# jiaw-z/DKT-Stereo

Hardware: AMD Instinct MI355X
Metric: stereo pairs/sec at 736x1248 D=192, 32 iters (RAFT-Stereo test_mode forward) (higher is better)
Workload: dtype f32 io/accumulate; convolution products = 3x fp16-split MFMA (22-bit operands); lookup / correlation exact fp32

## Files before the change

### dkt_stereo_amd/csrc/corr_feat.hip

```cpp
#include "dkt_common.h"
#include <cstdlib>
#include <type_traits>

typedef float cf_f32x16 __attribute__((ext_vector_type(16)));

struct CorrFeatArgs {
    DktPtrs skew;
    const float *coords_x;
    long coords_bstride;
    const float *w;
    const float *bias;
    float *out;
    long out_bstride;
    float *tap;
    long tap_bstride;
    long HW;
    int H, W1, W2, pitch, nseg, Cout, relu;
    float inv_wm1[DKT_MAX_LEVELS];
    char *out_c8;
    long out_c8_bs, out_c8_plane;
    int out_c8_Wp, out_c8_ch0;
    float act_scale;
};

// ... 178 lines not shown
    const long waves = (long)a.H * a.nseg;
    dim3 grid((unsigned)((waves + 3) / 4), (unsigned)B);
    if (a.Cout <= 32) hipLaunchKernelGGL((corr_feat_kernel<L, R, 1>), grid, dim3(256), 0, st, a);
    else hipLaunchKernelGGL((corr_feat_kernel<L, R, 2>), grid, dim3(256), 0, st, a);
    return dkt_launch_status();
}

typedef float cf_f32x4 __attribute__((ext_vector_type(4)));

template <int R, int MT>
__global__ __launch_bounds__(256) void corr_feat16_kernel(CorrFeatArgs a) {
    constexpr int K = 2 * R + 1;
    const int lane = threadIdx.x & 63;
    const int li = lane & 15, g = lane >> 4;
    const long gw = blockIdx.x * 4L + (threadIdx.x >> 6);
    const long hrow = gw / a.nseg;
    if (hrow >= a.H) return;
    const int seg0 = (int)(gw - hrow * a.nseg) * 16;
    const int w1 = seg0 + li;
    const bool live = w1 < a.W1;
    const int w1c = live ? w1 : a.W1 - 1;
    const int b = blockIdx.y;
    const long p = hrow * a.W1 + w1c;
    const float cx = a.coords_x[(size_t)b * a.coords_bstride + p];

    float A[MT][K];
#pragma unroll
    for (int s = 0; s < K; ++s)
#pragma unroll
        for (int m = 0; m < MT; ++m) {
            const int co = 16 * m + li;
            const bool ok = co < a.Cout;
            const float wv = a.w[(long)(g * K + s) * a.Cout + (ok ? co : 0)];
            A[m][s] = ok ? wv : 0.0f;
        }
    float bv[MT][4];
#pragma unroll
    for (int m = 0; m < MT; ++m)
#pragma unroll
        for (int r = 0; r < 4; ++r) bv[m][r] = 0.0f;
    if (a.bias) {
#pragma unroll
        for (int m = 0; m < MT; ++m)
#pragma unroll
            for (int r = 0; r < 4; ++r) {
                const int co = 16 * m + 4 * g + r;
                bv[m][r] = a.bias[co < a.Cout ? co : a.Cout - 1];
            }
    }

    const int lv = g;
    const int wi = a.W2 >> lv;
    const int qm = (w1c >> lv) % wi;
    const float *lvl = g == 0 ? a.skew.p[0] : g == 1 ? a.skew.p[1] : g == 2 ? a.skew.p[2] : a.skew.p[3];
    const float inv = g == 0 ? a.inv_wm1[0] : g == 1 ? a.inv_wm1[1] : g == 2 ? a.inv_wm1[2] : a.inv_wm1[3];
    const float *base = lvl + (((long)b * a.H + hrow) * wi) * (long)a.pitch + w1c;
    const float xc = __fdiv_rn(cx, (float)(1 << lv));
    const float wm1 = (float)(wi - 1);
    const float hwm1 = __fdiv_rn(wm1, 2.0f);
    DktTap taps[K];
#pragma unroll
    for (int k = 0; k < K; ++k) taps[k] = cf_tap(__fadd_rn((float)(k - R), xc), wm1, inv, hwm1);
    const int i0 = cf_clamp_idx(taps[0].fl, wi);
    float win[K + 1];
#pragma unroll
    for (int t = 0; t <= K; ++t) {
        const int c = i0 + t;
        const bool in = c >= 0 && c < wi;
        int sidx = (in ? c : 0) - qm;
        if (sidx < 0) sidx += wi;
        const float x = base[(long)sidx * a.pitch];
        win[t] = in ? x : 0.0f;
    }
    bool odd = false;
#pragma unroll
    for (int k = 0; k < K; ++k) odd |= cf_clamp_idx(taps[k].fl, wi) != i0 + k;
    float v[K];
#pragma unroll
    for (int k = 0; k < K; ++k) v[k] = dkt_blend(win[k], win[k + 1], taps[k]);
    if (__any(odd)) {
        auto at = [&](int c) -> float {
            if (c < 0 || c >= wi) return 0.0f;
            int sidx = c - qm;
            if (sidx < 0) sidx += wi;
            return base[(long)sidx * a.pitch];
        };
#pragma unroll
        for (int k = 0; k < K; ++k) {
            const int ik = cf_clamp_idx(taps[k].fl, wi);
            if (ik != i0 + k) v[k] = dkt_blend(at(ik), at(ik + 1), taps[k]);
        }
    }
    if (a.tap && live) {
        float *t = a.tap + (size_t)b * a.tap_bstride + p;
#pragma unroll
        for (int k = 0; k < K; ++k) t[(size_t)(g * K + k) * a.HW] = v[k];
    }

    cf_f32x4 acc[MT];
#pragma unroll
    for (int m = 0; m < MT; ++m)
#pragma unroll
        for (int r = 0; r < 4; ++r) {
            acc[m][r] = 0.0f;
            asm volatile("" ::"v"(bv[m][r]));
        }
#pragma unroll
    for (int s = 0; s < K; ++s)
#pragma unroll
        for (int m = 0; m < MT; ++m)
            acc[m] = __builtin_amdgcn_mfma_f32_16x16x4f32(A[m][s], v[s], acc[m], 0, 0, 0);

    const bool full = 16 * MT <= a.Cout && seg0 + 16 <= a.W1;
    if (a.out_c8) {
        char *pb = a.out_c8 + (size_t)b * a.out_c8_bs + ((size_t)(hrow + 1) * a.out_c8_Wp + (w1c + 1)) * 16;
#pragma unroll
        for (int m = 0; m < MT; ++m) {
            unsigned hw[2], lw[2];
#pragma unroll
            for (int d = 0; d < 2; ++d) {
                float y0 = __fadd_rn(acc[m][2 * d], bv[m][2 * d]), y1 = __fadd_rn(acc[m][2 * d + 1], bv[m][2 * d + 1]);
                if (a.relu) { y0 = dkt_relu(y0); y1 = dkt_relu(y1); }
                if (16 * m + 4 * g + 2 * d >= a.Cout) y0 = 0.0f;
                if (16 * m + 4 * g + 2 * d + 1 >= a.Cout) y1 = 0.0f;
                y0 *= a.act_scale; y1 *= a.act_scale;
                const _Float16 h0 = (_Float16)y0, h1 = (_Float16)y1;
                union { _Float16 h[2]; unsigned u; } t0, t1;
                t0.h[0] = h0; t0.h[1] = h1;
                t1.h[0] = (_Float16)(y0 - (float)h0); t1.h[1] = (_Float16)(y1 - (float)h1);
                hw[d] = t0.u; lw[d] = t1.u;
            }
            const bool even = (g & 1) == 0;
            const unsigned s0 = __shfl_xor(even ? lw[0] : hw[0], 16), s1 = __shfl_xor(even ? lw[1] : hw[1], 16);
            const uint4 v = even ? make_uint4(hw[0], hw[1], s0, s1) : make_uint4(s0, s1, lw[0], lw[1]);
            if (live) {
                const int grp = ((a.out_c8_ch0 + 16 * m) >> 3) + (g >> 1);
                *(uint4 *)(pb + (size_t)grp * 2 * a.out_c8_plane + (even ? 0 : a.out_c8_plane)) = v;
            }
        }
        return;
    }
    float *ob = a.out + (size_t)b * a.out_bstride + hrow * a.W1 + w1c;
#pragma unroll
    for (int m = 0; m < MT; ++m)
#pragma unroll
        for (int r = 0; r < 4; ++r) {
            const int co = 16 * m + 4 * g + r;
            float y = __fadd_rn(acc[m][r], bv[m][r]);
            if (a.relu) y = dkt_relu(y);
            if (full || (co < a.Cout && live)) ob[(size_t)co * a.HW] = y;
        }
}

template <int R, class CX>
__device__ __forceinline__ void corr_feat64_body(const CorrFeatArgs &a, long bx, int b, CX coord) {
    constexpr int K = 2 * R + 1;
    constexpr int VP = 12;
    static_assert((4 * K + 3) / 4 <= VP, "row pitch holds the k steps");
    __shared__ __attribute__((aligned(16))) float vs[4 * 64 * VP];
    const int lane = threadIdx.x & 63;
    const int g = __builtin_amdgcn_readfirstlane(threadIdx.x >> 6);
    const int nseg = (a.W1 + 63) / 64;
    const long hrow = bx / nseg;
    const int seg0 = (int)(bx - hrow * nseg) * 64;
    constexpr int NS = (4 * K) / 4;
    float Aw[NS];
    {
        const int j = lane & 15, q = lane >> 4;
        const int co = 16 * g + j;
#pragma unroll
        for (int sidx = 0; sidx < NS; ++sidx) {
            const int kk = 4 * sidx + q;
            const float wv = a.w[(long)kk * a.Cout + (co < a.Cout ? co : 0)];
            Aw[sidx] = co < a.Cout ? wv : 0.0f;
        }
    }
    {
        const int w1 = seg0 + lane;
        const bool live = w1 < a.W1;
        const int w1c = live ? w1 : a.W1 - 1;
        const long p = hrow * a.W1 + w1c;
        const float cx = coord(b, p, live, g);
        const int lv = g;
        const int wi = a.W2 >> lv;
        const int qm = (w1c >> lv) % wi;
        const float *lvl = a.skew.p[lv];
        const float inv = a.inv_wm1[lv];
        const float *base = lvl + (((long)b * a.H + hrow) * wi) * (long)a.pitch + w1c;
        const float xc = __fdiv_rn(cx, (float)(1 << lv));
        const float wm1 = (float)(wi - 1);
        const float hwm1 = __fdiv_rn(wm1, 2.0f);
        DktTap taps[K];
#pragma unroll
        for (int k = 0; k < K; ++k) taps[k] = cf_tap(__fadd_rn((float)(k - R), xc), wm1, inv, hwm1);
        const int i0 = cf_clamp_idx(taps[0].fl, wi);
        float win[K + 1];
#pragma unroll
        for (int t = 0; t <= K; ++t) {
            const int c = i0 + t;
            const bool in = c >= 0 && c < wi;
            int sidx = (in ? c : 0) - qm;
            if (sidx < 0) sidx += wi;
            const float x = base[(long)sidx * a.pitch];
            win[t] = in ? x : 0.0f;
        }
        bool odd = false;
#pragma unroll
        for (int k = 0; k < K; ++k) odd |= cf_clamp_idx(taps[k].fl, wi) != i0 + k;
        float v[K];
#pragma unroll
        for (int k = 0; k < K; ++k) v[k] = dkt_blend(win[k], win[k + 1], taps[k]);
        if (__any(odd)) {
            auto at = [&](int c) -> float {
                if (c < 0 || c >= wi) return 0.0f;
                int sidx = c - qm;
                if (sidx < 0) sidx += wi;
                return base[(long)sidx * a.pitch];
            };
#pragma unroll
            for (int k = 0; k < K; ++k) {
                const int ik = cf_clamp_idx(taps[k].fl, wi);
                if (ik != i0 + k) v[k] = dkt_blend(at(ik), at(ik + 1), taps[k]);
            }
        }
#pragma unroll
        for (int k = 0; k < K; ++k) vs[(((g * K + k) & 3) * 64 + lane) * VP + ((g * K + k) >> 2)] = v[k];
        if (a.tap && live) {
            float *t = a.tap + (size_t)b * a.tap_bstride + p;
#pragma unroll
            for (int k = 0; k < K; ++k) t[(size_t)(g * K + k) * a.HW] = v[k];
        }
    }
    __syncthreads();
    const int m = g;
    if (16 * m >= a.Cout) return;
    const int j = lane & 15, q = lane >> 4;
    typedef float f32x4_ __attribute__((ext_vector_type(4)));
    f32x4_ acc[4];
#pragma unroll
    for (int t = 0; t < 4; ++t) acc[t] = f32x4_{0.f, 0.f, 0.f, 0.f};
#pragma unroll
    for (int t0 = 0; t0 < 4; t0 += 2) {
        float bs[2][VP];
#pragma unroll
        for (int t = 0; t < 2; ++t) {
            const float4 *row = (const float4 *)(vs + (q * 64 + 16 * (t0 + t) + j) * VP);
#pragma unroll
            for (int i = 0; i < VP / 4; ++i) {
                const float4 f = row[i];
                bs[t][4 * i] = f.x; bs[t][4 * i + 1] = f.y; bs[t][4 * i + 2] = f.z; bs[t][4 * i + 3] = f.w;
            }
        }
#pragma unroll
        for (int sidx = 0; sidx < NS; ++sidx) {
#pragma unroll
            for (int t = 0; t < 2; ++t) acc[t0 + t] = __builtin_amdgcn_mfma_f32_16x16x4f32(Aw[sidx], bs[t][sidx], acc[t0 + t], 0, 0, 0);
        }
    }
    float bv[4];
#pragma unroll
    for (int r = 0; r < 4; ++r) {
        const int co = 16 * m + 4 * q + r;
        bv[r] = a.bias ? a.bias[co < a.Cout ? co : a.Cout - 1] : 0.0f;
    }
#pragma unroll
    for (int t = 0; t < 4; ++t) {
        const int w1 = seg0 + 16 * t + j;
        const bool live = w1 < a.W1;
        float y[4];
#pragma unroll
        for (int r = 0; r < 4; ++r) {
            y[r] = __fadd_rn(acc[t][r], bv[r]);
            if (a.relu) y[r] = dkt_relu(y[r]);
            if (16 * m + 4 * q + r >= a.Cout) y[r] = 0.0f;
        }
        if (a.out_c8) {
            unsigned hw[2], lw[2];
#pragma unroll
            for (int d = 0; d < 2; ++d) {
                const float y0 = y[2 * d] * a.act_scale, y1 = y[2 * d + 1] * a.act_scale;
                const _Float16 h0 = (_Float16)y0, h1 = (_Float16)y1;
                union { _Float16 h[2]; unsigned u; } t0, t1;
                t0.h[0] = h0; t0.h[1] = h1;
                t1.h[0] = (_Float16)(y0 - (float)h0); t1.h[1] = (_Float16)(y1 - (float)h1);
                hw[d] = t0.u; lw[d] = t1.u;
            }
            const bool even = (q & 1) == 0;
            const unsigned s0 = __shfl_xor(even ? lw[0] : hw[0], 16), s1 = __shfl_xor(even ? lw[1] : hw[1], 16);
            const uint4 v = even ? make_uint4(hw[0], hw[1], s0, s1) : make_uint4(s0, s1, lw[0], lw[1]);
            if (live) {
                const int grp = ((a.out_c8_ch0 + 16 * m) >> 3) + (q >> 1);
                char *pb = a.out_c8 + (size_t)b * a.out_c8_bs + ((size_t)(hrow + 1) * a.out_c8_Wp + (w1 + 1)) * 16;
                *(uint4 *)(pb + (size_t)grp * 2 * a.out_c8_plane + (even ? 0 : a.out_c8_plane)) = v;
            }
        } else if (live) {
            float *ob = a.out + (size_t)b * a.out_bstride + hrow * a.W1 + w1;
#pragma unroll
            for (int r = 0; r < 4; ++r) {
                const int co = 16 * m + 4 * q + r;
                if (co < a.Cout) ob[(size_t)co * a.HW] = y[r];
            }
        }
    }
}

template <int R>
__global__ __launch_bounds__(256, 8) void corr_feat64_kernel(CorrFeatArgs a) {
    corr_feat64_body<R>(a, (long)blockIdx.x, (int)blockIdx.y,
                        [&](int b, long p, bool, int) -> float { return a.coords_x[(size_t)b * a.coords_bstride + p]; });
}

#include "stem7_body.h"

struct FrontArgs {
    CorrFeatArgs cf;
    Stem7Args s7;
    const float *planes; long planes_bs; int n_co;
    const float *head_bias;
    const float *x_old; long x_old_bs;
    float *x_new; long x_new_bs;
    const float *x0; long x0_bs;
    float *flow; long flow_bs;
    int nb_stem;
};

__device__ __forceinline__ float front_coord(const FrontArgs &f, int b, int oh, int ow, long p) {
    const int H = f.cf.H, W = f.cf.W1;
    const long HW = f.cf.HW;
    float s = 0.0f;
    for (int cb = 0; cb < f.n_co; ++cb) {
        const float *pl = f.planes + (long)b * f.planes_bs + (long)cb * 9 * HW;
#pragma unroll
        for (int t = 0; t < 9; ++t) {
            const int ih = oh + t / 3 - 1, iw = ow + t % 3 - 1;
            const bool in = ih >= 0 && ih < H && iw >= 0 && iw < W;
            const float v = pl[(long)t * HW + (in ? (long)ih * W + iw : 0)];
            s = __fadd_rn(s, in ? v : 0.0f);
        }
    }
    s = __fadd_rn(s, f.head_bias ? f.head_bias[0] : 0.0f);
    return __fadd_rn(f.x_old[(long)b * f.x_old_bs + p], s);
}

template <int R>
__global__ __launch_bounds__(256) void motion_front_kernel(FrontArgs f) {
    const int b = blockIdx.y;
    if ((int)blockIdx.x < f.nb_stem) {
        const long HW = f.cf.HW;
        const float *fl = f.flow + (long)b * f.flow_bs;
        const float *x0 = f.x0 + (long)b * f.x0_bs;
        stem7_tile(f.s7, (int)(blockIdx.x / f.s7.n_co), (int)(blockIdx.x % f.s7.n_co), b, [&](int ih, int iw, long off, float (&v)[4]) {
            v[0] = __fsub_rn(front_coord(f, b, ih, iw, off), x0[off]);
#pragma unroll
            for (int c = 1; c < 4; ++c) v[c] = fl[(long)(c < f.s7.Cin ? c : 0) * HW + off];
        });
        return;
    }
    corr_feat64_body<R>(f.cf, (long)blockIdx.x - f.nb_stem, b, [&](int bb, long p, bool live, int g) -> float {
        const int oh = (int)(p / f.cf.W1), ow = (int)(p - (long)oh * f.cf.W1);
        const float nx = front_coord(f, bb, oh, ow, p);
        if (g == 0 && live) {
            f.x_new[(long)bb * f.x_new_bs + p] = nx;
            f.flow[(long)bb * f.flow_bs + p] = __fsub_rn(nx, f.x0[(long)bb * f.x0_bs + p]);
        }
        return nx;
    });
}

template <int R>
static int cf16_launch(CorrFeatArgs a, int B, hipStream_t st) {
    a.nseg = (a.W1 + 15) / 16;
    const long waves = (long)a.H * a.nseg;
    dim3 grid((unsigned)((waves + 3) / 4), (unsigned)B);
    switch ((a.Cout + 15) / 16) {
        case 1: hipLaunchKernelGGL((corr_feat16_kernel<R, 1>), grid, dim3(256), 0, st, a); break;
        case 2: hipLaunchKernelGGL((corr_feat16_kernel<R, 2>), grid, dim3(256), 0, st, a); break;
        case 3: hipLaunchKernelGGL((corr_feat16_kernel<R, 3>), grid, dim3(256), 0, st, a); break;
        default: hipLaunchKernelGGL((corr_feat16_kernel<R, 4>), grid, dim3(256), 0, st, a); break;
    }
    return dkt_launch_status();
}

static int corr_feat_impl(const float *const *skew, const float *coords_x, long coords_bstride,
                          const float *weight, const float *bias, float *out, long out_bstride,
                          float *tap, long tap_bstride, void *out_c8, long out_c8_bstride_bytes, int out_c8_ch0, float act_scale,
                          int B, int H, int W1, int W2, int L, int r, int Cout, int relu,
                          int device, void *stream) {
    if (!skew || !coords_x || !weight || (!out && !out_c8)) return DKT_E_NULL;
    if (out_c8 && (L != 4 || (out_c8_ch0 & 7) || !(act_scale > 0.0f))) return DKT_E_UNSUPPORTED;
    if (B <= 0 || H <= 0 || W1 <= 0 || W2 <= 0 || B > 65535 || Cout <= 0) return DKT_E_SHAPE;
    if (L < 1 || L > DKT_MAX_LEVELS || (W2 >> (L - 1)) == 0) return DKT_E_LEVELS;
    if (r < 0 || r > DKT_MAX_RADIUS) return DKT_E_RADIUS;
    if (Cout > 64 || !((L == 4 || L == 2 || L == 3) && (r == 4 || r == 3))) return DKT_E_UNSUPPORTED;
    if ((W2 >> (L - 1)) < 2) return DKT_E_UNSUPPORTED;
    CorrFeatArgs a;
    for (int i = 0; i < DKT_MAX_LEVELS; ++i) {
        a.skew.p[i] = i < L ? skew[i] : nullptr;
        if (i < L && !skew[i]) return DKT_E_NULL;
        const int wi = i < L ? (W2 >> i) : 0;
        a.inv_wm1[i] = wi > 1 ? (float)(1.0 / (double)(wi - 1)) : 0.0f;
    }
    a.coords_x = coords_x;
    a.coords_bstride = coords_bstride;
    a.w = weight;
    a.bias = bias;
    a.out = out;
    a.out_bstride = out_bstride;
    a.tap = tap;
    a.tap_bstride = tap_bstride;
    a.HW = (long)H * W1;
    a.H = H; a.W1 = W1; a.W2 = W2;
    a.pitch = (W1 + 31) & ~31;
    a.nseg = (W1 + 31) / 32;
    a.Cout = Cout;
    a.relu = relu ? 1 : 0;
    int Hp = 0, Wp = 0;
    dkt_act_c8_dims(H, W1, &Hp, &Wp);
    a.out_c8 = (char *)out_c8; a.out_c8_bs = out_c8_bstride_bytes; a.out_c8_plane = (long)Hp * Wp * 16;
    a.out_c8_Wp = Wp; a.out_c8_ch0 = out_c8_ch0; a.act_scale = act_scale;
    DKT_ENTER(device);
    hipStream_t st = (hipStream_t)stream;
    if (L == 4) {
        const long blocks = (long)H * ((W1 + 63) / 64);
        if (blocks > 0x7fffffffL) return DKT_E_SHAPE;
        dim3 grid((unsigned)blocks, (unsigned)B);
        if (r == 4) hipLaunchKernelGGL(corr_feat64_kernel<4>, grid, dim3(256), 0, st, a);
        else hipLaunchKernelGGL(corr_feat64_kernel<3>, grid, dim3(256), 0, st, a);
        return dkt_launch_status();
    }
    if (out_c8) return r == 4 ? cf16_launch<4>(a, B, st) : cf16_launch<3>(a, B, st);
    if (r == 4) {
        if (L == 4) return cf_launch<4, 4>(a, B, st);
        if (L == 3) return cf_launch<3, 4>(a, B, st);
        return cf_launch<2, 4>(a, B, st);
    }
    if (L == 4) return cf_launch<4, 3>(a, B, st);
    if (L == 3) return cf_launch<3, 3>(a, B, st);
    return cf_launch<2, 3>(a, B, st);
}

extern "C" int dkt_corr1d_lookup_conv1x1(const float *const *skew, const float *coords_x, long coords_bstride,
                                         const float *weight, const float *bias, float *out, long out_bstride,
                                         float *tap, long tap_bstride,
                                         int B, int H, int W1, int W2, int L, int r, int Cout, int relu,
                                         int device, void *stream) {
    if (!out) return DKT_E_NULL;
    return corr_feat_impl(skew, coords_x, coords_bstride, weight, bias, out, out_bstride, tap, tap_bstride, nullptr, 0, 0, 1.0f,
                          B, H, W1, W2, L, r, Cout, relu, device, stream);
}

extern "C" int dkt_corr1d_lookup_conv1x1_c8(const float *const *skew, const float *coords_x, long coords_bstride,
                                            const float *weight, const float *bias, void *out_c8, long out_c8_bstride_bytes,
                                            int out_c8_ch0, float act_scale, int B, int H, int W1, int W2, int L, int r, int Cout,
                                            int relu, int device, void *stream) {
    if (!out_c8) return DKT_E_NULL;
    return corr_feat_impl(skew, coords_x, coords_bstride, weight, bias, nullptr, 0, nullptr, 0, out_c8, out_c8_bstride_bytes,
                          out_c8_ch0, act_scale, B, H, W1, W2, L, r, Cout, relu, device, stream);
}

extern "C" int dkt_motion_front_c8(const dkt_motion_front_desc *d, int device, void *stream) {
    if (!d) return DKT_E_NULL;
    if (!d->skew || !d->planes || !d->x_old || !d->x_new || !d->x0 || !d->flow || !d->w_cor || !d->cor_c8 || !d->stem_w_hi ||
        !d->stem_w_lo || !d->flo_c8)
        return DKT_E_NULL;
    if (d->x_new == d->x_old) return DKT_E_SHAPE;
    const int B = d->B, H = d->H, W1 = d->W1, W2 = d->W2, L = d->L, r = d->r;
    if (B <= 0 || H <= 0 || W1 <= 0 || W2 <= 0 || B > 65535 || d->n_co < 1) return DKT_E_SHAPE;
    if (L != 4 || (r != 4 && r != 3) || d->cor_channels <= 0 || d->cor_channels > 64 || (W2 >> (L - 1)) < 2) return DKT_E_UNSUPPORTED;
    if (d->stem_cin < 1 || d->stem_cin > 4 || d->stem_cout <= 0) return DKT_E_SHAPE;
    if ((d->cor_c8_ch0 & 7) || (d->flo_c8_ch0 & 7) || !(d->cor_act_scale > 0.0f) || !(d->flo_act_scale > 0.0f) ||
        !(d->stem_in_scale > 0.0f) || !(d->stem_out_scale > 0.0f))
        return DKT_E_SHAPE;
    FrontArgs f;
    CorrFeatArgs &a = f.cf;
    for (int i = 0; i < DKT_MAX_LEVELS; ++i) {
        a.skew.p[i] = i < L ? d->skew[i] : nullptr;
        if (i < L && !d->skew[i]) return DKT_E_NULL;
        const int wi = i < L ? (W2 >> i) : 0;
        a.inv_wm1[i] = wi > 1 ? (float)(1.0 / (double)(wi - 1)) : 0.0f;
    }
    a.coords_x = nullptr; a.coords_bstride = 0;
    a.w = d->w_cor; a.bias = d->b_cor;
    a.out = nullptr; a.out_bstride = 0; a.tap = nullptr; a.tap_bstride = 0;
    a.HW = (long)H * W1;
    a.H = H; a.W1 = W1; a.W2 = W2;
    a.pitch = (W1 + 31) & ~31;
    a.nseg = (W1 + 31) / 32;
    a.Cout = d->cor_channels;
    a.relu = 1;
    int Hp = 0, Wp = 0;
    dkt_act_c8_dims(H, W1, &Hp, &Wp);
    a.out_c8 = (char *)d->cor_c8; a.out_c8_bs = d->cor_c8_bstride_bytes; a.out_c8_plane = (long)Hp * Wp * 16;
    a.out_c8_Wp = Wp; a.out_c8_ch0 = d->cor_c8_ch0; a.act_scale = d->cor_act_scale;
    Stem7Args &s = f.s7;
    s.x = nullptr; s.x_bs = 0;
    s.whi = (const _Float16 *)d->stem_w_hi; s.wlo = (const _Float16 *)d->stem_w_lo;
    s.bias = d->stem_bias; s.out_scale = d->stem_out_scale; s.in_scale = d->stem_in_scale;
    s.y = nullptr; s.y_bs = 0;
    s.Cin = d->stem_cin; s.Cout = d->stem_cout; s.CoutPad = (d->stem_cout + 63) & ~63;
    s.H = H; s.W = W1;
    s.tiles_w = (W1 + 31) / 32;
    s.tiles_xy = s.tiles_w * ((H + 3) / 4);
    s.n_co = s.CoutPad / 64;
    s.relu = 1;
    s.y_c8 = (char *)d->flo_c8; s.y_c8_bs = d->flo_c8_bstride_bytes; s.y_c8_plane = (long)Hp * Wp * 16; s.y_c8_Wp = Wp;
    s.y_c8_ch0 = d->flo_c8_ch0; s.act_scale = d->flo_act_scale;
    f.planes = d->planes; f.planes_bs = d->planes_bstride; f.n_co = d->n_co;
    f.head_bias = d->head_bias;
    f.x_old = d->x_old; f.x_old_bs = d->x_old_bstride;
    f.x_new = d->x_new; f.x_new_bs = d->x_new_bstride;
    f.x0 = d->x0; f.x0_bs = d->x0_bstride;
    f.flow = d->flow; f.flow_bs = d->flow_bstride;
    const long nb_stem = (long)s.tiles_xy * s.n_co, nb_look = (long)H * ((W1 + 63) / 64);
    if (nb_stem + nb_look > 0x7fffffffL) return DKT_E_SHAPE;
    f.nb_stem = (int)nb_stem;
    DKT_ENTER(device);
    dim3 grid((unsigned)(nb_stem + nb_look), (unsigned)B);
    if (r == 4) hipLaunchKernelGGL(motion_front_kernel<4>, grid, dim3(256), 0, (hipStream_t)stream, f);
    else hipLaunchKernelGGL(motion_front_kernel<3>, grid, dim3(256), 0, (hipStream_t)stream, f);
// ... 3 lines not shown
```

### dkt_stereo_amd/csrc/resample_c8.hip

```cpp
#include "resample.h"

__device__ __forceinline__ unsigned rs_pack_h2(_Float16 a, _Float16 b) {
    union { _Float16 h[2]; unsigned u; } v;
    v.h[0] = a;
    v.h[1] = b;
    return v.u;
}

__device__ __forceinline__ void rs_store_c8(char *p, long plane, const float (&v)[8], float scale) {
    unsigned hw[4], lw[4];
#pragma unroll
    for (int d = 0; d < 4; ++d) {
        const float x0 = v[2 * d] * scale, x1 = v[2 * d + 1] * scale;
        const _Float16 a0 = (_Float16)x0, a1 = (_Float16)x1;
        hw[d] = rs_pack_h2(a0, a1);
        lw[d] = rs_pack_h2((_Float16)(x0 - (float)a0), (_Float16)(x1 - (float)a1));
    }
    *(uint4 *)p = make_uint4(hw[0], hw[1], hw[2], hw[3]);
    *(uint4 *)(p + plane) = make_uint4(lw[0], lw[1], lw[2], lw[3]);
}

__device__ __forceinline__ void pool2x_c8_body(const float *__restrict__ x, long x_bs, char *__restrict__ dst, long dst_bs,
                                               int C, int H, int W, int Ho, int Wo, int Wp, long plane, int ch0, float scale,
                                               int bx, int oy, int bz) {
    const int ox = bx * 128 + threadIdx.x;
    const int g = bz % ((C + 7) / 8), b = bz / ((C + 7) / 8);
    if (ox >= Wo) return;
    const float *xb = x + (long)b * x_bs;
    float v[8];
#pragma unroll
    for (int k = 0; k < 8; ++k) {
        const int c = g * 8 + k;
        float t[9];
        dkt_pool9_load(xb + (long)(c < C ? c : C - 1) * H * W, H, W, oy, ox, t);
        const float avg = dkt_pool9_avg(t);
        v[k] = c < C ? avg : 0.0f;
    }
    rs_store_c8(dst + (long)b * dst_bs + (long)((ch0 >> 3) + g) * 2 * plane + ((long)(oy + 1) * Wp + (ox + 1)) * 16, plane, v, scale);
}

__device__ __forceinline__ void interp_c8_body(const float *__restrict__ x, long x_bs, char *__restrict__ dst, long dst_bs,
                                               int C, int H, int W, int Ho, int Wo, float sy, float sx, int Wp, long plane,
                                               int ch0, float scale, int bx, int oy, int bz) {
    const int ox = bx * 128 + threadIdx.x;
    const int g = bz % ((C + 7) / 8), b = bz / ((C + 7) / 8);
    if (ox >= Wo) return;
    const DktLerp ty = dkt_lerp(oy, sy, H), tx = dkt_lerp(ox, sx, W);
    const float *xb = x + (long)b * x_bs;
    float a0[8], a1[8], b0[8], b1[8];
#pragma unroll
    for (int k = 0; k < 8; ++k) {
        const int c = g * 8 + k;
        const float *p = xb + (long)(c < C ? c : C - 1) * H * W;
        a0[k] = p[(long)ty.i0 * W + tx.i0]; a1[k] = p[(long)ty.i0 * W + tx.i1];
        b0[k] = p[(long)ty.i1 * W + tx.i0]; b1[k] = p[(long)ty.i1 * W + tx.i1];
    }
    float v[8];
#pragma unroll
    for (int k = 0; k < 8; ++k) {
        const float o = dkt_lerp_blend(ty, tx, a0[k], a1[k], b0[k], b1[k]);
        v[k] = g * 8 + k < C ? o : 0.0f;
    }
    rs_store_c8(dst + (long)b * dst_bs + (long)((ch0 >> 3) + g) * 2 * plane + ((long)(oy + 1) * Wp + (ox + 1)) * 16, plane, v, scale);
}

__global__ __launch_bounds__(128) void pool2x_c8_kernel(const float *__restrict__ x, long x_bs, char *__restrict__ dst, long dst_bs,
                                                        int C, int H, int W, int Ho, int Wo, int Wp, long plane, int ch0, float scale) {
    pool2x_c8_body(x, x_bs, dst, dst_bs, C, H, W, Ho, Wo, Wp, plane, ch0, scale, blockIdx.x, blockIdx.y, blockIdx.z);
}

__global__ __launch_bounds__(128) void interp_c8_kernel(const float *__restrict__ x, long x_bs, char *__restrict__ dst, long dst_bs,
                                                        int C, int H, int W, int Ho, int Wo, float sy, float sx, int Wp, long plane,
                                                        int ch0, float scale) {
    interp_c8_body(x, x_bs, dst, dst_bs, C, H, W, Ho, Wo, sy, sx, Wp, plane, ch0, scale, blockIdx.x, blockIdx.y, blockIdx.z);
}

struct RsJob {
    const float *x; long x_bs;
    char *dst; long dst_bs;
    int C, H, W, Ho, Wo, Wp; long plane; int ch0; float scale;
    float sy, sx;
    int kind;
    int nbx, nby;
};
struct RsPair { RsJob j[2]; };

__global__ __launch_bounds__(128) void resample_pair_c8_kernel(RsPair a, int nb0) {
    const bool second = (int)blockIdx.x >= nb0;
    const RsJob &j = a.j[second ? 1 : 0];
    int id = (int)blockIdx.x - (second ? nb0 : 0);
    const int bx = id % j.nbx; id /= j.nbx;
    const int oy = id % j.nby, bz = id / j.nby;
    if (j.kind == 0) pool2x_c8_body(j.x, j.x_bs, j.dst, j.dst_bs, j.C, j.H, j.W, j.Ho, j.Wo, j.Wp, j.plane, j.ch0, j.scale, bx, oy, bz);
    else interp_c8_body(j.x, j.x_bs, j.dst, j.dst_bs, j.C, j.H, j.W, j.Ho, j.Wo, j.sy, j.sx, j.Wp, j.plane, j.ch0, j.scale, bx, oy, bz);
}

static int rs_fill(RsJob &j, const dkt_resample_c8_job *d, long &blocks) {
    if (!d || !d->x || !d->dst) return DKT_E_NULL;
    if (d->B <= 0 || d->C <= 0 || d->H <= 0 || d->W <= 0 || (d->ch0 & 7) || !(d->scale > 0.0f)) return DKT_E_SHAPE;
    if (d->kind != 0 && d->kind != 1) return DKT_E_UNSUPPORTED;
    j.x = d->x; j.x_bs = d->x_bstride; j.dst = (char *)d->dst; j.dst_bs = d->dst_bstride_bytes;
    j.C = d->C; j.H = d->H; j.W = d->W; j.ch0 = d->ch0; j.scale = d->scale; j.kind = d->kind;
    if (d->kind == 0) {
        j.Ho = (d->H - 1) / 2 + 1; j.Wo = (d->W - 1) / 2 + 1;
        j.sy = j.sx = 0.0f;
    } else {
        if (d->Ho <= 0 || d->Wo <= 0) return DKT_E_SHAPE;
        j.Ho = d->Ho; j.Wo = d->Wo;
        j.sy = j.Ho > 1 ? (float)(d->H - 1) / (float)(j.Ho - 1) : 0.0f;
        j.sx = j.Wo > 1 ? (float)(d->W - 1) / (float)(j.Wo - 1) : 0.0f;
    }
    int Hp, Wp;
    dkt_act_c8_dims(j.Ho, j.Wo, &Hp, &Wp);
    j.Wp = Wp; j.plane = (long)Hp * Wp * 16;
    j.nbx = (j.Wo + 127) / 128; j.nby = j.Ho;
    blocks = (long)j.nbx * j.nby * d->B * ((d->C + 7) / 8);
    return DKT_OK;
}

extern "C" int dkt_resample_pair_c8(const dkt_resample_c8_job *job0, const dkt_resample_c8_job *job1, int device, void *stream) {
    RsPair a;
    long n0 = 0, n1 = 0;
    int rc = rs_fill(a.j[0], job0, n0);
    if (rc != DKT_OK) return rc;
    rc = rs_fill(a.j[1], job1, n1);
    if (rc != DKT_OK) return rc;
    if (n0 + n1 > 0x7fffffffL) return DKT_E_SHAPE;
    DKT_ENTER(device);
    hipLaunchKernelGGL(resample_pair_c8_kernel, dim3((unsigned)(n0 + n1)), dim3(128), 0, (hipStream_t)stream, a, (int)n0);
    return dkt_launch_status();
}

extern "C" int dkt_pool2x_c8(const float *x, long x_bstride, void *dst, long dst_bstride_bytes, int B, int C, int H, int W,
                             int ch0, float scale, int device, void *stream) {
    if (!x || !dst) return DKT_E_NULL;
    if (B <= 0 || C <= 0 || H <= 0 || W <= 0 || (ch0 & 7) || !(scale > 0.0f)) return DKT_E_SHAPE;
    const int Ho = (H - 1) / 2 + 1, Wo = (W - 1) / 2 + 1;
    int Hp, Wp;
    dkt_act_c8_dims(Ho, Wo, &Hp, &Wp);
    const long gz = (long)B * ((C + 7) / 8);
    if (gz > 65535 || Ho > 65535) return DKT_E_SHAPE;
    DKT_ENTER(device);
    hipLaunchKernelGGL(pool2x_c8_kernel, dim3((unsigned)((Wo + 127) / 128), (unsigned)Ho, (unsigned)gz), dim3(128), 0, (hipStream_t)stream,
                       x, x_bstride, (char *)dst, dst_bstride_bytes, C, H, W, Ho, Wo, Wp, (long)Hp * Wp * 16, ch0, scale);
    return dkt_launch_status();
}

extern "C" int dkt_interp_c8(const float *x, long x_bstride, void *dst, long dst_bstride_bytes, int B, int C, int H, int W,
                             int Ho, int Wo, int ch0, float scale, int device, void *stream) {
    if (!x || !dst) return DKT_E_NULL;
    if (B <= 0 || C <= 0 || H <= 0 || W <= 0 || Ho <= 0 || Wo <= 0 || (ch0 & 7) || !(scale > 0.0f)) return DKT_E_SHAPE;
    int Hp, Wp;
    dkt_act_c8_dims(Ho, Wo, &Hp, &Wp);
    const long gz = (long)B * ((C + 7) / 8);
    if (gz > 65535 || Ho > 65535) return DKT_E_SHAPE;
    const float sy = Ho > 1 ? (float)(H - 1) / (float)(Ho - 1) : 0.0f;
    const float sx = Wo > 1 ? (float)(W - 1) / (float)(Wo - 1) : 0.0f;
    DKT_ENTER(device);
    hipLaunchKernelGGL(interp_c8_kernel, dim3((unsigned)((Wo + 127) / 128), (unsigned)Ho, (unsigned)gz), dim3(128), 0, (hipStream_t)stream,
                       x, x_bstride, (char *)dst, dst_bstride_bytes, C, H, W, Ho, Wo, sy, sx, Wp, (long)Hp * Wp * 16, ch0, scale);
    return dkt_launch_status();
}
```

### dkt_stereo_amd/csrc/stem7_body.h

```cpp
#pragma once
#include "dkt_common.h"

typedef _Float16 s7_f16x8 __attribute__((ext_vector_type(8)));
typedef _Float16 s7_f16x4 __attribute__((ext_vector_type(4)));
typedef float s7_f32x16 __attribute__((ext_vector_type(16)));

#define S7_STEPS 14

struct Stem7Args {
    const float *x;
    long x_bs;
    const _Float16 *whi, *wlo;
    const float *bias;
    float out_scale, in_scale;
    float *y;
    long y_bs;
    int Cin, Cout, CoutPad, H, W, tiles_w, tiles_xy, n_co;
    int relu;
    char *y_c8;
    long y_c8_bs, y_c8_plane;
    int y_c8_Wp, y_c8_ch0;
    float act_scale;
};

template <class LD>
__device__ __forceinline__ void stem7_tile(const Stem7Args &a, int t, int cb, int b, LD load) {
    constexpr int TR = 4, PR = TR + 6, PC = 40;
    __shared__ __attribute__((aligned(16))) _Float16 phi[PR * PC * 4], plo[PR * PC * 4];
    const int tid = threadIdx.x, lane = tid & 63, wave = tid >> 6;
    const int li = lane & 31, kg = lane >> 5;
    const int w0 = (t % a.tiles_w) * 32, h0 = (t / a.tiles_w) * TR;
    const long HW = (long)a.H * a.W;
    for (int pp = tid; pp < PR * PC; pp += 256) {
        const int pr = pp / PC, pc = pp - pr * PC;
        const int ih = h0 - 3 + pr, iw = w0 - 3 + pc;
        const bool ok = ih >= 0 && ih < a.H && iw >= 0 && iw < a.W;
        const long off = ok ? (long)ih * a.W + iw : 0;
        s7_f16x4 hv, lv;
        float in[4];
        load(ok ? ih : 0, ok ? iw : 0, off, in);
#pragma unroll
        for (int c = 0; c < 4; ++c) {
            float v = (ok && c < a.Cin) ? in[c] : 0.0f;
            v *= a.in_scale;
            const _Float16 h = (_Float16)v;
            hv[c] = h;
            lv[c] = (_Float16)(v - (float)h);
        }
        *(s7_f16x4 *)(phi + pp * 4) = hv;
        *(s7_f16x4 *)(plo + pp * 4) = lv;
    }
    __syncthreads();
    s7_f32x16 acc[2];
#pragma unroll
    for (int m = 0; m < 2; ++m)
#pragma unroll
        for (int r = 0; r < 16; ++r) acc[m][r] = 0.0f;
    const int co0 = cb * 64;
    const _Float16 *wh = a.whi + ((long)(co0 + li)) * 16 + kg * 8;
    const _Float16 *wl = a.wlo + ((long)(co0 + li)) * 16 + kg * 8;
    const long wstep = (long)a.CoutPad * 16;
#pragma unroll
    for (int s = 0; s < S7_STEPS; ++s) {
        const int dy = s >> 1, half = s & 1;
        s7_f16x8 Ah[2], Al[2];
#pragma unroll
        for (int m = 0; m < 2; ++m) {
            Ah[m] = *(const s7_f16x8 *)(wh + s * wstep + m * 32 * 16);
            Al[m] = *(const s7_f16x8 *)(wl + s * wstep + m * 32 * 16);
        }
        const int pp = (wave + dy) * PC + li + 4 * half + 2 * kg;
        union { s7_f16x8 v; s7_f16x4 h[2]; } Bh, Bl;
        Bh.h[0] = *(const s7_f16x4 *)(phi + pp * 4);
        Bh.h[1] = *(const s7_f16x4 *)(phi + pp * 4 + 4);
        Bl.h[0] = *(const s7_f16x4 *)(plo + pp * 4);
        Bl.h[1] = *(const s7_f16x4 *)(plo + pp * 4 + 4);
#pragma unroll
        for (int m = 0; m < 2; ++m) {
            acc[m] = __builtin_amdgcn_mfma_f32_32x32x16_f16(Ah[m], Bh.v, acc[m], 0, 0, 0);
            acc[m] = __builtin_amdgcn_mfma_f32_32x32x16_f16(Al[m], Bh.v, acc[m], 0, 0, 0);
            acc[m] = __builtin_amdgcn_mfma_f32_32x32x16_f16(Ah[m], Bl.v, acc[m], 0, 0, 0);
        }
    }
    const int oh = h0 + wave, ow = w0 + li;
    const bool inside = oh < a.H && ow < a.W;
    float *yo = a.y ? a.y + (long)b * a.y_bs + (long)(inside ? oh : 0) * a.W + (inside ? ow : 0) : nullptr;
#pragma unroll
    for (int m = 0; m < 2; ++m) {
        float v[16];
#pragma unroll
        for (int r = 0; r < 16; ++r) {
            const int co = co0 + m * 32 + 4 * kg + (r & 3) + 8 * (r >> 2);
            float t = acc[m][r] * a.out_scale + (a.bias ? a.bias[co < a.Cout ? co : a.Cout - 1] : 0.0f);
            if (a.relu) t = dkt_relu(t);
            v[r] = co < a.Cout ? t : 0.0f;
            if (yo && inside && co < a.Cout) yo[(long)co * HW] = v[r];
        }
        if (a.y_c8) {
#pragma unroll
            for (int jp = 0; jp < 2; ++jp) {
                unsigned ha[2], la[2], hb[2], lb[2];
#pragma unroll
                for (int d = 0; d < 2; ++d) {
                    const float x0 = v[8 * jp + 2 * d] * a.act_scale, x1 = v[8 * jp + 2 * d + 1] * a.act_scale;
                    const float y0 = v[8 * jp + 4 + 2 * d] * a.act_scale, y1 = v[8 * jp + 4 + 2 * d + 1] * a.act_scale;
                    const _Float16 a0 = (_Float16)x0, a1 = (_Float16)x1, b0 = (_Float16)y0, b1 = (_Float16)y1;
                    union { _Float16 h[2]; unsigned u; } t0, t1, t2, t3;
                    t0.h[0] = a0; t0.h[1] = a1;
                    t1.h[0] = (_Float16)(x0 - (float)a0); t1.h[1] = (_Float16)(x1 - (float)a1);
                    t2.h[0] = b0; t2.h[1] = b1;
                    t3.h[0] = (_Float16)(y0 - (float)b0); t3.h[1] = (_Float16)(y1 - (float)b1);
                    ha[d] = t0.u; la[d] = t1.u; hb[d] = t2.u; lb[d] = t3.u;
                }
#pragma unroll
                for (int d = 0; d < 2; ++d) {
                    auto r = __builtin_amdgcn_permlane32_swap(ha[d], hb[d], false, false);
                    ha[d] = r[0]; hb[d] = r[1];
                    auto q = __builtin_amdgcn_permlane32_swap(la[d], lb[d], false, false);
                    la[d] = q[0]; lb[d] = q[1];
                }
                if (inside) {
                    const int g = ((a.y_c8_ch0 + co0 + m * 32) >> 3) + 2 * jp + kg;
                    char *p = a.y_c8 + (long)b * a.y_c8_bs + (long)g * 2 * a.y_c8_plane + ((long)(oh + 1) * a.y_c8_Wp + (ow + 1)) * 16;
                    *(uint4 *)p = make_uint4(ha[0], ha[1], hb[0], hb[1]);
                    *(uint4 *)(p + a.y_c8_plane) = make_uint4(la[0], la[1], lb[0], lb[1]);
                }
            }
        }
    }
}
```

Measured before the change: 33.52.

## Share front-kernel LDS, split coord conv across waves, vectorize pool resample

In motion_front_kernel, the 3x3 plane-sum coordinate computation is now split across the four waves, with each wave loading a subset of taps into shared memory before every wave sums them. Before this, every wave recomputed all taps on its own. The stem patch and the corr sample buffer now use a single shared LDS allocation, and occupancy is hinted with launch_bounds(256,5). The resample pool kernel gains a float4-vectorized path that produces two outputs per thread, and both resample kernels now use flat 1D chunked indexing. The cost of this is added __syncthreads barriers in the corr path and extra code paths for aligned and unaligned inputs.

```diff
diff --git a/dkt_stereo_amd/csrc/corr_feat.hip b/dkt_stereo_amd/csrc/corr_feat.hip
--- a/dkt_stereo_amd/csrc/corr_feat.hip
+++ b/dkt_stereo_amd/csrc/corr_feat.hip
@@ -354,12 +354,12 @@
         }
 }
 
+#define CF64_VS_FLOATS (4 * 64 * 12)
 template <int R, class CX>
-__device__ __forceinline__ void corr_feat64_body(const CorrFeatArgs &a, long bx, int b, CX coord) {
+__device__ __forceinline__ void corr_feat64_body(const CorrFeatArgs &a, long bx, int b, CX coord, float *vs) {
     constexpr int K = 2 * R + 1;
     constexpr int VP = 12;
-    static_assert((4 * K + 3) / 4 <= VP, "row pitch holds the k steps");
-    __shared__ __attribute__((aligned(16))) float vs[4 * 64 * VP];
+    static_assert((4 * K + 3) / 4 <= VP && 4 * 64 * VP == CF64_VS_FLOATS, "row pitch holds the k steps");
     const int lane = threadIdx.x & 63;
     const int g = __builtin_amdgcn_readfirstlane(threadIdx.x >> 6);
     const int nseg = (a.W1 + 63) / 64;
@@ -382,7 +382,7 @@
         const bool live = w1 < a.W1;
         const int w1c = live ? w1 : a.W1 - 1;
         const long p = hrow * a.W1 + w1c;
-        const float cx = coord(b, p, live, g);
+        const float cx = coord(b, p, live, g, vs);
         const int lv = g;
         const int wi = a.W2 >> lv;
         const int qm = (w1c >> lv) % wi;
@@ -508,8 +508,9 @@
 
 template <int R>
 __global__ __launch_bounds__(256, 8) void corr_feat64_kernel(CorrFeatArgs a) {
+    __shared__ __attribute__((aligned(16))) float vs[CF64_VS_FLOATS];
     corr_feat64_body<R>(a, (long)blockIdx.x, (int)blockIdx.y,
-                        [&](int b, long p, bool, int) -> float { return a.coords_x[(size_t)b * a.coords_bstride + p]; });
+                        [&](int b, long p, bool, int, float *) -> float { return a.coords_x[(size_t)b * a.coords_bstride + p]; }, vs);
 }
 
 #include "stem7_body.h"
@@ -544,8 +545,49 @@
     return __fadd_rn(f.x_old[(long)b * f.x_old_bs + p], s);
 }
 
+#define FRONT_CB 4
+static_assert(FRONT_CB * 9 * 64 <= CF64_VS_FLOATS, "a pass fits the sample buffer of corr_feat64_body");
+
+__device__ __forceinline__ float front_coord_block(const FrontArgs &f, int b, long p, int g, float *vs) {
+    const int H = f.cf.H, W = f.cf.W1, lane = threadIdx.x & 63;
+    const long HW = f.cf.HW;
+    const int oh = (int)(p / W), ow = (int)(p - (long)oh * W);
+    const float xo = f.x_old[(long)b * f.x_old_bs + p];
+    const float hb = f.head_bias ? f.head_bias[0] : 0.0f;
+    float s = 0.0f;
+    for (int cb0 = 0; cb0 < f.n_co; cb0 += FRONT_CB) {
+        const int ncb = f.n_co - cb0 < FRONT_CB ? f.n_co - cb0 : FRONT_CB;
+        const float *pl = f.planes + (long)b * f.planes_bs + (long)cb0 * 9 * HW;
+        float u[FRONT_CB * 9 / 4];
+#pragma unroll
+        for (int j = 0; j < FRONT_CB * 9 / 4; ++j) {
+            const int i = g + 4 * j;
+            const int t = i % 9;
+            const int ih = oh + t / 3 - 1, iw = ow + t % 3 - 1;
+            const bool in = i < ncb * 9 && ih >= 0 && ih < H && iw >= 0 && iw < W;
+            const float v = pl[(long)(i < ncb * 9 ? i : 0) * HW + (in ? (long)ih * W + iw : 0)];
+            u[j] = in ? v : 0.0f;
+        }
+#pragma unroll
+        for (int j = 0; j < FRONT_CB * 9 / 4; ++j) vs[(g + 4 * j) * 64 + lane] = u[j];
+        __syncthreads();
+        for (int cb = 0; cb < ncb; ++cb) {
+            float t[9];
+#pragma unroll
+            for (int k = 0; k < 9; ++k) t[k] = vs[(cb * 9 + k) * 64 + lane];
+#pragma unroll
+            for (int k = 0; k < 9; ++k) s = __fadd_rn(s, t[k]);
+        }
+        __syncthreads();
+    }
+    s = __fadd_rn(s, hb);
+    return __fadd_rn(xo, s);
+}
+
 template <int R>
-__global__ __launch_bounds__(256) void motion_front_kernel(FrontArgs f) {
+__global__ __launch_bounds__(256, 5) void motion_front_kernel(FrontArgs f) {
+    static_assert(S7_PATCH_HALVES * 2 <= CF64_VS_FLOATS * 4, "the stem patch fits the sample buffer");
+    __shared__ __attribute__((aligned(16))) float lds[CF64_VS_FLOATS];
     const int b = blockIdx.y;
     if ((int)blockIdx.x < f.nb_stem) {
         const long HW = f.cf.HW;
@@ -555,18 +597,18 @@
             v[0] = __fsub_rn(front_coord(f, b, ih, iw, off), x0[off]);
 #pragma unroll
             for (int c = 1; c < 4; ++c) v[c] = fl[(long)(c < f.s7.Cin ? c : 0) * HW + off];
-        });
+        }, (_Float16 *)lds);
         return;
     }
-    corr_feat64_body<R>(f.cf, (long)blockIdx.x - f.nb_stem, b, [&](int bb, long p, bool live, int g) -> float {
-        const int oh = (int)(p / f.cf.W1), ow = (int)(p - (long)oh * f.cf.W1);
-        const float nx = front_coord(f, bb, oh, ow, p);
+    corr_feat64_body<R>(f.cf, (long)blockIdx.x - f.nb_stem, b, [&](int bb, long p, bool live, int g, float *vs) -> float {
+        const float x0 = f.x0[(long)bb * f.x0_bs + p];
+        const float nx = front_coord_block(f, bb, p, g, vs);
         if (g == 0 && live) {
             f.x_new[(long)bb * f.x_new_bs + p] = nx;
-            f.flow[(long)bb * f.flow_bs + p] = __fsub_rn(nx, f.x0[(long)bb * f.x0_bs + p]);
+            f.flow[(long)bb * f.flow_bs + p] = __fsub_rn(nx, x0);
         }
         return nx;
-    });
+    }, lds);
 }
 
 template <int R>
diff --git a/dkt_stereo_amd/csrc/resample_c8.hip b/dkt_stereo_amd/csrc/resample_c8.hip
--- a/dkt_stereo_amd/csrc/resample_c8.hip
+++ b/dkt_stereo_amd/csrc/resample_c8.hip
@@ -20,12 +20,20 @@
     *(uint4 *)(p + plane) = make_uint4(lw[0], lw[1], lw[2], lw[3]);
 }
 
+__device__ __forceinline__ bool rs_item(int chunk, int Hy, int Wx, int &oy, int &ox) {
+    const unsigned n = (unsigned)chunk * 128u + threadIdx.x;
+    if (n >= (unsigned)Hy * (unsigned)Wx) return false;
+    oy = (int)(n / (unsigned)Wx);
+    ox = (int)(n - (unsigned)oy * (unsigned)Wx);
+    return true;
+}
+
 __device__ __forceinline__ void pool2x_c8_body(const float *__restrict__ x, long x_bs, char *__restrict__ dst, long dst_bs,
                                                int C, int H, int W, int Ho, int Wo, int Wp, long plane, int ch0, float scale,
-                                               int bx, int oy, int bz) {
-    const int ox = bx * 128 + threadIdx.x;
+                                               int chunk, int bz) {
+    int oy, ox;
+    if (!rs_item(chunk, Ho, Wo, oy, ox)) return;
     const int g = bz % ((C + 7) / 8), b = bz / ((C + 7) / 8);
-    if (ox >= Wo) return;
     const float *xb = x + (long)b * x_bs;
     float v[8];
 #pragma unroll
@@ -35,16 +43,49 @@
         dkt_pool9_load(xb + (long)(c < C ? c : C - 1) * H * W, H, W, oy, ox, t);
         const float avg = dkt_pool9_avg(t);
         v[k] = c < C ? avg : 0.0f;
+        if (k & 1) __builtin_amdgcn_sched_barrier(0);
     }
     rs_store_c8(dst + (long)b * dst_bs + (long)((ch0 >> 3) + g) * 2 * plane + ((long)(oy + 1) * Wp + (ox + 1)) * 16, plane, v, scale);
+}
+
+__device__ __forceinline__ void pool2x_c8_body4(const float *__restrict__ x, long x_bs, char *__restrict__ dst, long dst_bs,
+                                                int C, int H, int W, int Ho, int Wo, int Wp, long plane, int ch0, float scale,
+                                                int chunk, int bz) {
+    int oy, oj;
+    if (!rs_item(chunk, Ho, Wo >> 1, oy, oj)) return;
+    const int g = bz % ((C + 7) / 8), b = bz / ((C + 7) / 8);
+    const float *xb = x + (long)b * x_bs;
+    const int iy0 = 2 * oy - 1;
+    const bool top = iy0 >= 0, bot = iy0 + 2 < H, left = oj > 0;
+    const int r0 = (top ? iy0 : 0) * W + 4 * oj, r1 = (iy0 + 1) * W + 4 * oj, r2 = (bot ? iy0 + 2 : 0) * W + 4 * oj;
+    const int lo = left ? -1 : 0;
+    float v0[8], v1[8];
+#pragma unroll
+    for (int k = 0; k < 8; ++k) {
+        const int c = g * 8 + k;
+        const float *p = xb + (long)(c < C ? c : C - 1) * H * W;
+        const float4 m0 = *(const float4 *)(p + r0), m1 = *(const float4 *)(p + r1), m2 = *(const float4 *)(p + r2);
+        const float l0 = p[r0 + lo], l1 = p[r1 + lo], l2 = p[r2 + lo];
+        const float z = 0.0f;
+        const float t0[9] = {top && left ? l0 : z, top ? m0.x : z, top ? m0.y : z, left ? l1 : z, m1.x, m1.y,
+                             bot && left ? l2 : z, bot ? m2.x : z, bot ? m2.y : z};
+        const float t1[9] = {top ? m0.y : z, top ? m0.z : z, top ? m0.w : z, m1.y, m1.z, m1.w, bot ? m2.y : z, bot ? m2.z : z, bot ? m2.w : z};
+        const float a0 = dkt_pool9_avg(t0), a1 = dkt_pool9_avg(t1);
+        v0[k] = c < C ? a0 : 0.0f;
+        v1[k] = c < C ? a1 : 0.0f;
+        if (k & 1) __builtin_amdgcn_sched_barrier(0);
+    }
+    char *o = dst + (long)b * dst_bs + (long)((ch0 >> 3) + g) * 2 * plane + ((long)(oy + 1) * Wp + (2 * oj + 1)) * 16;
+    rs_store_c8(o, plane, v0, scale);
+    rs_store_c8(o + 16, plane, v1, scale);
 }
 
 __device__ __forceinline__ void interp_c8_body(const float *__restrict__ x, long x_bs, char *__restrict__ dst, long dst_bs,
                                                int C, int H, int W, int Ho, int Wo, float sy, float sx, int Wp, long plane,
-                                               int ch0, float scale, int bx, int oy, int bz) {
-    const int ox = bx * 128 + threadIdx.x;
+                                               int ch0, float scale, int chunk, int bz) {
+    int oy, ox;
+    if (!rs_item(chunk, Ho, Wo, oy, ox)) return;
     const int g = bz % ((C + 7) / 8), b = bz / ((C + 7) / 8);
-    if (ox >= Wo) return;
     const DktLerp ty = dkt_lerp(oy, sy, H), tx = dkt_lerp(ox, sx, W);
     const float *xb = x + (long)b * x_bs;
     float a0[8], a1[8], b0[8], b1[8];
@@ -62,17 +103,6 @@
         v[k] = g * 8 + k < C ? o : 0.0f;
     }
     rs_store_c8(dst + (long)b * dst_bs + (long)((ch0 >> 3) + g) * 2 * plane + ((long)(oy + 1) * Wp + (ox + 1)) * 16, plane, v, scale);
-}
-
-__global__ __launch_bounds__(128) void pool2x_c8_kernel(const float *__restrict__ x, long x_bs, char *__restrict__ dst, long dst_bs,
-                                                        int C, int H, int W, int Ho, int Wo, int Wp, long plane, int ch0, float scale) {
-    pool2x_c8_body(x, x_bs, dst, dst_bs, C, H, W, Ho, Wo, Wp, plane, ch0, scale, blockIdx.x, blockIdx.y, blockIdx.z);
-}
-
-__global__ __launch_bounds__(128) void interp_c8_kernel(const float *__restrict__ x, long x_bs, char *__restrict__ dst, long dst_bs,
-                                                        int C, int H, int W, int Ho, int Wo, float sy, float sx, int Wp, long plane,
-                                                        int ch0, float scale) {
-    interp_c8_body(x, x_bs, dst, dst_bs, C, H, W, Ho, Wo, sy, sx, Wp, plane, ch0, scale, blockIdx.x, blockIdx.y, blockIdx.z);
 }
 
 struct RsJob {
@@ -81,18 +111,31 @@
     int C, H, W, Ho, Wo, Wp; long plane; int ch0; float scale;
     float sy, sx;
     int kind;
-    int nbx, nby;
+    int vec;
+    int nchunk;
 };
+
+__device__ __forceinline__ void rs_run(const RsJob &j, int id) {
+    const int chunk = id % j.nchunk, bz = id / j.nchunk;
+    if (j.kind == 0) {
+        if (j.vec) pool2x_c8_body4(j.x, j.x_bs, j.dst, j.dst_bs, j.C, j.H, j.W, j.Ho, j.Wo, j.Wp, j.plane, j.ch0, j.scale, chunk, bz);
+        else pool2x_c8_body(j.x, j.x_bs, j.dst, j.dst_bs, j.C, j.H, j.W, j.Ho, j.Wo, j.Wp, j.plane, j.ch0, j.scale, chunk, bz);
+    } else {
+        interp_c8_body(j.x, j.x_bs, j.dst, j.dst_bs, j.C, j.H, j.W, j.Ho, j.Wo, j.sy, j.sx, j.Wp, j.plane, j.ch0, j.scale, chunk, bz);
+    }
+}
+
+__global__ __launch_bounds__(128) void resample_c8_kernel(RsJob j) { rs_run(j, (int)blockIdx.x); }
+
 struct RsPair { RsJob j[2]; };
 
 __global__ __launch_bounds__(128) void resample_pair_c8_kernel(RsPair a, int nb0) {
     const bool second = (int)blockIdx.x >= nb0;
-    const RsJob &j = a.j[second ? 1 : 0];
-    int id = (int)blockIdx.x - (second ? nb0 : 0);
-    const int bx = id % j.nbx; id /= j.nbx;
-    const int oy = id % j.nby, bz = id / j.nby;
-    if (j.kind == 0) pool2x_c8_body(j.x, j.x_bs, j.dst, j.dst_bs, j.C, j.H, j.W, j.Ho, j.Wo, j.Wp, j.plane, j.ch0, j.scale, bx, oy, bz);
-    else interp_c8_body(j.x, j.x_bs, j.dst, j.dst_bs, j.C, j.H, j.W, j.Ho, j.Wo, j.sy, j.sx, j.Wp, j.plane, j.ch0, j.scale, bx, oy, bz);
+    rs_run(a.j[second ? 1 : 0], (int)blockIdx.x - (second ? nb0 : 0));
+}
+
+static bool rs_pool_vec(const float *x, long x_bs, int H, int W) {
+    return (W & 3) == 0 && (x_bs & 3) == 0 && ((uintptr_t)x & 15) == 0 && (long)H * W <= 0x7fffffffL;
 }
 
 static int rs_fill(RsJob &j, const dkt_resample_c8_job *d, long &blocks) {
@@ -113,8 +156,11 @@
     int Hp, Wp;
     dkt_act_c8_dims(j.Ho, j.Wo, &Hp, &Wp);
     j.Wp = Wp; j.plane = (long)Hp * Wp * 16;
-    j.nbx = (j.Wo + 127) / 128; j.nby = j.Ho;
-    blocks = (long)j.nbx * j.nby * d->B * ((d->C + 7) / 8);
+    j.vec = d->kind == 0 && rs_pool_vec(d->x, d->x_bstride, d->H, d->W) ? 1 : 0;
+    const long items = (long)j.Ho * (j.vec ? j.Wo >> 1 : j.Wo);
+    if (items > 0x7fffff00L) return DKT_E_SHAPE;
+    j.nchunk = (int)((items + 127) / 128);
+    blocks = (long)j.nchunk * d->B * ((d->C + 7) / 8);
     return DKT_OK;
 }
 
@@ -131,33 +177,25 @@
     return dkt_launch_status();
 }
 
+static int rs_single(const dkt_resample_c8_job &d, int device, void *stream) {
+    RsJob j;
+    long n = 0;
+    const int rc = rs_fill(j, &d, n);
+    if (rc != DKT_OK) return rc;
+    if (n > 0x7fffffffL) return DKT_E_SHAPE;
+    DKT_ENTER(device);
+    hipLaunchKernelGGL(resample_c8_kernel, dim3((unsigned)n), dim3(128), 0, (hipStream_t)stream, j);
+    return dkt_launch_status();
+}
+
 extern "C" int dkt_pool2x_c8(const float *x, long x_bstride, void *dst, long dst_bstride_bytes, int B, int C, int H, int W,
                              int ch0, float scale, int device, void *stream) {
-    if (!x || !dst) return DKT_E_NULL;
-    if (B <= 0 || C <= 0 || H <= 0 || W <= 0 || (ch0 & 7) || !(scale > 0.0f)) return DKT_E_SHAPE;
-    const int Ho = (H - 1) / 2 + 1, Wo = (W - 1) / 2 + 1;
-    int Hp, Wp;
-    dkt_act_c8_dims(Ho, Wo, &Hp, &Wp);
-    const long gz = (long)B * ((C + 7) / 8);
-    if (gz > 65535 || Ho > 65535) return DKT_E_SHAPE;
-    DKT_ENTER(device);
-    hipLaunchKernelGGL(pool2x_c8_kernel, dim3((unsigned)((Wo + 127) / 128), (unsigned)Ho, (unsigned)gz), dim3(128), 0, (hipStream_t)stream,
-                       x, x_bstride, (char *)dst, dst_bstride_bytes, C, H, W, Ho, Wo, Wp, (long)Hp * Wp * 16, ch0, scale);
-    return dkt_launch_status();
+    dkt_resample_c8_job d = {x, x_bstride, dst, dst_bstride_bytes, B, C, H, W, 0, 0, ch0, 0, scale};
+    return rs_single(d, device, stream);
 }
 
 extern "C" int dkt_interp_c8(const float *x, long x_bstride, void *dst, long dst_bstride_bytes, int B, int C, int H, int W,
                              int Ho, int Wo, int ch0, float scale, int device, void *stream) {
-    if (!x || !dst) return DKT_E_NULL;
-    if (B <= 0 || C <= 0 || H <= 0 || W <= 0 || Ho <= 0 || Wo <= 0 || (ch0 & 7) || !(scale > 0.0f)) return DKT_E_SHAPE;
-    int Hp, Wp;
-    dkt_act_c8_dims(Ho, Wo, &Hp, &Wp);
-    const long gz = (long)B * ((C + 7) / 8);
-    if (gz > 65535 || Ho > 65535) return DKT_E_SHAPE;
-    const float sy = Ho > 1 ? (float)(H - 1) / (float)(Ho - 1) : 0.0f;
-    const float sx = Wo > 1 ? (float)(W - 1) / (float)(Wo - 1) : 0.0f;
-    DKT_ENTER(device);
-    hipLaunchKernelGGL(interp_c8_kernel, dim3((unsigned)((Wo + 127) / 128), (unsigned)Ho, (unsigned)gz), dim3(128), 0, (hipStream_t)stream,
-                       x, x_bstride, (char *)dst, dst_bstride_bytes, C, H, W, Ho, Wo, sy, sx, Wp, (long)Hp * Wp * 16, ch0, scale);
-    return dkt_launch_status();
-}
+    dkt_resample_c8_job d = {x, x_bstride, dst, dst_bstride_bytes, B, C, H, W, Ho, Wo, ch0, 1, scale};
+    return rs_single(d, device, stream);
+}
diff --git a/dkt_stereo_amd/csrc/stem7_body.h b/dkt_stereo_amd/csrc/stem7_body.h
--- a/dkt_stereo_amd/csrc/stem7_body.h
+++ b/dkt_stereo_amd/csrc/stem7_body.h
@@ -23,10 +23,12 @@
     float act_scale;
 };
 
+#define S7_PATCH_HALVES (2 * (4 + 6) * 40 * 4)
 template <class LD>
-__device__ __forceinline__ void stem7_tile(const Stem7Args &a, int t, int cb, int b, LD load) {
+__device__ __forceinline__ void stem7_tile(const Stem7Args &a, int t, int cb, int b, LD load, _Float16 *patch) {
     constexpr int TR = 4, PR = TR + 6, PC = 40;
-    __shared__ __attribute__((aligned(16))) _Float16 phi[PR * PC * 4], plo[PR * PC * 4];
+    static_assert(2 * PR * PC * 4 == S7_PATCH_HALVES, "patch size");
+    _Float16 *phi = patch, *plo = patch + PR * PC * 4;
     const int tid = threadIdx.x, lane = tid & 63, wave = tid >> 6;
     const int li = lane & 31, kg = lane >> 5;
     const int w0 = (t % a.tiles_w) * 32, h0 = (t / a.tiles_w) * TR;
@@ -129,3 +131,9 @@
         }
     }
 }
+
+template <class LD>
+__device__ __forceinline__ void stem7_tile(const Stem7Args &a, int t, int cb, int b, LD load) {
+    __shared__ __attribute__((aligned(16))) _Float16 patch[S7_PATCH_HALVES];
+    stem7_tile(a, t, cb, b, load, patch);
+}
```

Result: no change. 33.79, median of 6 (+0.8%).
